# megvii-research/OccDepth

Measured on AMD Instinct MI355X. Metric: frames/sec forward, SemanticKITTI stereo->256x256x32 voxels, higher is better.
Workload: dtype f32 storage and accumulate; matrix arithmetic as 3x bf16 split (hi + mid + lo of both operands, six v_mfma_f32_32x32x16_bf16 per K step; error vs float64 tested within 1.5x of the exact-fp32 kernels', measured 0.8-1.1x) in the head convolutions (K2s3), the small-volume 3x3x3 convolutions and transpo

## Files before the change

include/occdepth_amd.h:

```cpp
#ifndef OCCDEPTH_AMD_H
#define OCCDEPTH_AMD_H

#include <stdint.h>

#ifdef __cplusplus
extern "C" {
#endif

#define OCCD_OK 0
#define OCCD_EINVAL (-1)
#define OCCD_ELAUNCH (-2)
#define OCCD_ENOMEM (-3)

#define OCCD_MAX_VIEWS 4
#define OCCD_MAX_SCALES 4

#define OCCD_ACT_NONE 0
#define OCCD_ACT_RELU 1
#define OCCD_ACT_SIGMOID 2
#define OCCD_ACT_RELU_PRE 3

#define OCCD_ABI_VERSION 22
int occd_abi_version(void);
const char* occd_strerror(int code);
// ... 214 lines not shown
                       float* y, int32_t batch, int32_t C, int32_t H, int32_t W, int32_t k,
                       int32_t stride, int32_t pad_top, int32_t pad_left, int32_t Ho, int32_t Wo,
                       int32_t act, void* stream);
int occd_stem_conv3x3_nchw(const float* x, const float* w, const float* scale, const float* shift, float* y,
                           int32_t batch, int32_t H, int32_t W, int32_t cout, int32_t stride, int32_t pad_top,
                           int32_t pad_left, int32_t Ho, int32_t Wo, int32_t act, void* stream);
int occd_upsample_bilinear_cat_nchw(const float* x, const float* skip, float* out, int32_t batch,
                                    int32_t C, int32_t Cskip, int32_t h, int32_t w, int32_t H,
                                    int32_t W, void* stream);
int occd_upsample_bilinear_cat_nhwc(const float* x, const float* skip, float* out, int32_t batch, int32_t C, int32_t Cskip,
                                    int32_t h, int32_t w, int32_t H, int32_t W, void* stream);
int occd_upsample_bilinear_cat_nhwc_rows(const float* x, const float* skip, float* out, int32_t batch, int32_t C, int32_t Cskip,
                                         int32_t h, int32_t w, int32_t H, int32_t W, int32_t out_cs, void* stream);
int occd_upsample_bilinear_nhwc_bwd(const float* gout, float* gx, int32_t batch, int32_t C, int32_t gout_cs, int32_t h,
                                    int32_t w, int32_t H, int32_t W, void* stream);

int occd_upconv_gather_nchw(const float* z, float* out, int32_t batch, int32_t Cout, int32_t h, int32_t w,
                            int32_t H, int32_t W, int64_t z_channel_stride, int64_t z_batch_stride, void* stream);

int occd_upconv_gather_skip_nchw(const float* z, const float* skip, const float* wskip, const float* shift, float* out,
                                 int32_t batch, int32_t Cout, int32_t Cs, int32_t h, int32_t w, int32_t H, int32_t W,
                                 int64_t z_channel_stride, int64_t z_batch_stride, float slope, void* stream);

int occd_wino_input_transform_nchw(const float* x, float* V, int32_t batch, int32_t Cin, int32_t H, int32_t W,
                                   int32_t ty0, int32_t ths, void* stream);
int occd_wino_output_transform_nchw(const float* M, const float* scale, const float* shift, const float* res,
                                    float* y, int32_t batch, int32_t Cout, int32_t H, int32_t W, int32_t ty0,
                                    int32_t ths, int32_t act, float slope, int32_t res_first, void* stream);

int occd_wino_input_transform_cm(const float* x, float* Vt, int32_t batch, int32_t Cin, int32_t H, int32_t W,
                                 int64_t Tp, void* stream);
int occd_wino_output_transform_cm(const float* Mt, const float* scale, const float* shift, const float* res,
                                  float* y, int32_t batch, int32_t Cout, int32_t H, int32_t W, int64_t Tp,
                                  int32_t act, float slope, int32_t res_first, void* stream);

typedef struct occd_wino_args {
    const float* x;
    const float* upk;
    const float* shift;
    const float* res;
    float* y;
    int32_t batch, cin, cout, H, W;
    int32_t act, res_first, tile_hint;
    float slope;
} occd_wino_args;
int64_t occd_wino_packed_floats(int32_t cout, int32_t cin);
int occd_wino_pack_weights(const float* w, const float* scale, float* upk, int32_t cout, int32_t cin, void* stream);
int occd_wino_conv3x3_fwd(const occd_wino_args* a, void* stream);

int64_t occd_wino_packed_f16x2_bytes(int32_t cout, int32_t cin);
int occd_wino_pack_weights_f16x2(const float* w, const float* scale, void* upk, int32_t cout, int32_t cin, void* stream);
int occd_wino_conv3x3_f16x2_fwd(const occd_wino_args* a, void* stream);
int occd_wino_conv3x3_f16x2_fwd_ex(const occd_wino_args* a, int32_t max_workgroups, void* stream);

int occd_dwconv2d_bwd_data_nchw(const float* gy, const float* w, float* dx, int32_t batch, int32_t C, int32_t H,
                                int32_t W, int32_t k, int32_t stride, int32_t pad_top, int32_t pad_left, int32_t Ho,
                                int32_t Wo, void* stream);
int64_t occd_dwconv2d_bwd_weight_workspace_floats(int32_t batch, int32_t C, int32_t k, int32_t Ho, int32_t Wo);
int occd_dwconv2d_bwd_weight_nchw(const float* x, const float* gy, float* dw, float* workspace, int32_t batch, int32_t C,
                                  int32_t H, int32_t W, int32_t k, int32_t stride, int32_t pad_top, int32_t pad_left,
                                  int32_t Ho, int32_t Wo, void* stream);
int32_t occd_dwconv2d_pool_blocks(int32_t Ho, int32_t Wo);
int occd_dwconv2d_pool_nchw(const float* x, const float* w, const float* scale, const float* shift, float* y,
                            float* pool_part, int32_t batch, int32_t C, int32_t H, int32_t W, int32_t k,
                            int32_t stride, int32_t pad_top, int32_t pad_left, int32_t Ho, int32_t Wo,
                            int32_t act, int64_t x_plane_stride, void* stream);
int32_t occd_dwconv2d_set_stage(int32_t form);
int occd_plane_reduce(const float* a, const float* b, float* out, int64_t planes, int64_t S, void* stream);
int occd_se_bwd(const float* gg, const float* gate, const float* sums, const float* r, const float* w_reduce,
                const float* b_reduce, const float* w_expand, float* dz_scratch, float* gm, float* gw_reduce,
                float* gb_reduce, float* gw_expand, float* gb_expand, int32_t batch, int32_t C, int32_t Cr, int64_t S,
                void* stream);
int occd_depthnet_gate(const float* sps, const float* intrins, int64_t intr_stride, float factor, const float* w1,
                       const float* b1, const float* w2, const float* b2, const float* wr, const float* br,
                       const float* we, const float* be, float* gate, int32_t images, int32_t C, void* stream);
int occd_se_gate(const float* pool_part, const float* w_reduce, const float* b_reduce, const float* w_expand,
                 const float* b_expand, float* r_scratch, float* gate, int32_t batch, int32_t C, int32_t Cr,
                 int32_t nblk, int64_t S, void* stream);
int32_t occd_se_gate_set_fused(int32_t on);

int occd_graph_replace_memsets(void* graph);

typedef struct occd_pw_args {
    const float* x;
    const float* wpk;
    const float* shift;
    const float* gate;
    const float* res;
    float* y;
    int64_t N;
    int32_t batch, cin, cout;
    int32_t act, tile_hint;
    float slope;
    int32_t out_nhwc_cs;
} occd_pw_args;
int64_t occd_pw_packed_floats(int32_t cout, int32_t cin);
int occd_pw_pack_weights(const float* w, const float* scale, float* wpk, int32_t cout, int32_t cin, void* stream);
int occd_pw_conv_fwd(const occd_pw_args* a, void* stream);

int occd_argmax_channels(const float* x, int64_t rows, int32_t cs, int32_t coff, int32_t C,
                         const uint16_t* lut, uint16_t* out, void* stream);

#define OCCD_RENDER_MAX_VIEWS 8
typedef struct OccdRenderView {
    float o0[3], ou[3], ov[3];
    float d0[3], du[3], dv[3];
// ... 617 lines not shown
```

occdepth_amd/csrc/wino_conv2d.hip:

```cpp
#include <atomic>
#include <type_traits>
#include <vector>
#include "device.h"

namespace {

struct WinoP {
    const float* x;
    const float* upk;
    const float* shift;
    const float* res;
    float* y;
    int B, Cin, Cout, H, W;
    int chunks, nblk, wg_ty, wg_tx, nwg;
    int act, res_first;
    float slope;
};

constexpr uint32_t kWinoOutside = 0xFFFFFFF0u;
__device__ __forceinline__ float wino_acc_read(float a) {
    float t;
    asm volatile("v_accvgpr_read_b32 %0, %1" : "=v"(t) : "a"(a));
    return t;
}
// ... 295 lines not shown
    if (i >= total) return;
    const int j = i & 3, lane = (i >> 2) & 63;
    long t = i >> 8;
    const int blk = t % nblk; t /= nblk;
    const int rec = t & 15;
    const int chunk = (int)(t >> 4);
    const int q = rec >> 2, hh = (rec >> 1) & 1, part = rec & 1;
    const int xi = 8 * hh + 4 * part + j;
    const int co = blk * 32 + (lane & 31), ci = chunk * 8 + (lane >> 5) * 4 + q;
    float out = 0.f;
    if (co < cout && ci < cin) {
        const double G[4][3] = {{1, 0, 0}, {0.5, 0.5, 0.5}, {0.5, -0.5, 0.5}, {0, 0, 1}};
        const float* g = w + ((size_t)co * cin + ci) * 9;
        const int a = xi >> 2, bcol = xi & 3;
        double s = 0.0;
#pragma unroll
        for (int m = 0; m < 3; ++m)
#pragma unroll
            for (int n = 0; n < 3; ++n) s += G[a][m] * (double)g[m * 3 + n] * G[bcol][n];
        if (scale != nullptr) s *= (double)scale[co];
        out = (float)s;
    }
    upk[i] = out;
}

constexpr int kWinoStageExp = 1;
typedef _Float16 f16x2 __attribute__((ext_vector_type(2)));

struct WinoHP {
    const float* x;
    const uint16_t* upk;
    const float* fac;
    const float* shift;
    const float* res;
    float* y;
    int B, Cin, Cout, H, W;
    int chunks, nblk, wg_ty, wg_tx, nwg;
    int act, res_first;
    float slope;
};

__device__ __forceinline__ void split2_f16x2(float a, float b, uint32_t& hi, uint32_t& lo) {
    asm("" : "+v"(a));
    asm("" : "+v"(b));
    const f16x2 h = __builtin_convertvector((f32x2){a, b}, f16x2);
    float r0 = __builtin_fmaf((float)h[0], -2048.f, a * 2048.f);
    float r1 = __builtin_fmaf((float)h[1], -2048.f, b * 2048.f);
    asm("" : "+v"(r0));
    asm("" : "+v"(r1));
    hi = __builtin_bit_cast(uint32_t, h);
    lo = __builtin_bit_cast(uint32_t, __builtin_convertvector((f32x2){r0, r1}, f16x2));
}

template <int TWV, bool PERSIST, bool WE>
__global__ void __launch_bounds__(512, 2) wino3x3_f16x2_kernel(const WinoHP p) {
    constexpr int RW = 32 / TWV;
    constexpr int WGR = 4 * RW;
    constexpr int PR = 2 * WGR + 2;
    constexpr int PC = 2 * TWV + 2;
    constexpr int RS = TWV == 16 ? 48 : 68;
    constexpr int PLANE = PR * RS;
    constexpr int NEL = 8 * PLANE;
    constexpr int NDMA = (NEL + 511) / 512;
    constexpr int PBUF = NDMA * 512;
    constexpr int UOFF = 4 * PBUF;
    constexpr int XOFF = PERSIST ? 2 * PBUF : 0;
    constexpr int XFLOATS = 4 * 2 * 64 * 64 / (PERSIST ? 2 : 1);
    static_assert(XOFF + XFLOATS <= (PERSIST ? UOFF + 32 * 256 : 4 * 2 * 64 * 64), "the exchange must fit in the staging buffers");
    static_assert((UOFF + 32 * 256) * 4 <= 160 * 1024 && (XOFF + XFLOATS) * 4 <= 160 * 1024, "LDS of a CU");
    static_assert(XOFF % 4 == 0, "16-byte aligned exchange");
    extern __shared__ __attribute__((aligned(16))) float lds[];

    const size_t plane_hw = (size_t)p.H * p.W;
    const size_t u_rec = (size_t)p.nblk * 512;
    uint32_t voff[NDMA];
    int nb, b, ty0, tx0;
    auto fresh_tid = [] {
        int t = threadIdx.x;
        asm volatile("" : "+v"(t));
        return t;
    };
    const int wave = __builtin_amdgcn_readfirstlane(threadIdx.x >> 6);
    const int pr = wave & 3, h = wave >> 2;
    const bool h0 = h == 0;

    auto setup = [&](uint32_t v) {
        const uint32_t bid = xcd_remap(v, p.nwg);
        nb = bid % p.nblk;
        uint32_t t = bid / p.nblk;
        const int bx = t % p.wg_tx;
        t /= p.wg_tx;
        const int by = t % p.wg_ty;
        b = t / p.wg_ty;
        ty0 = by * WGR, tx0 = bx * TWV;
        const int gy0 = 2 * ty0 - 1, gx0 = 2 * tx0 - 1;
        const int lane = fresh_tid() & 63;
#pragma unroll
        for (int i = 0; i < NDMA; ++i) {
            const int e = (wave * NDMA + i) * 64 + lane;
            const int cin = e / PLANE, rem = e - cin * PLANE;
            const int row = rem / RS, col = rem - row * RS;
            const int gy = gy0 + row, gx = gx0 + col;
            const bool ok = e < NEL && col < PC && (unsigned)gy < (unsigned)p.H && (unsigned)gx < (unsigned)p.W;
            voff[i] = ok ? (uint32_t)((cin * plane_hw + (size_t)gy * p.W + gx) * 4) : 0xFFFFFFF0u;
        }
    };
    auto issue_patch = [&](int c, bool live = true) {
        const float* const xb = p.x + (size_t)b * p.Cin * plane_hw;
#pragma unroll
        for (int s = 0; s < 2; ++s) {
            const int ch0 = c * 16 + s * 8, left = live ? p.Cin - ch0 : 0;
            const auto rsrc = __builtin_amdgcn_make_buffer_rsrc((void*)(xb + (size_t)(left > 0 ? ch0 : 0) * plane_hw), 0,
                                                                left > 0 ? (uint32_t)((size_t)left * plane_hw * 4) : 0u, 0x00020000);
            float* pdst = lds + ((c & 1) * 2 + s) * PBUF + wave * NDMA * 64;
#pragma unroll
            for (int i = 0; i < NDMA; ++i)
                __builtin_amdgcn_raw_ptr_buffer_load_lds(rsrc, pdst + i * 64, 4, voff[i], 0, 0, 0);
        }
    };

    asm volatile("" ::"a"(0.f));
    f32x16 acc[8];

    static_assert(kWinoStageExp == 1, "the transform below stages 2 V");
    auto row_v = [&](auto hc, auto ic, const float* pl, uint32_t (&vh)[4][4], uint32_t (&vl)[4][4]) {
        constexpr int H = decltype(hc)::value, I = decltype(ic)::value;
        constexpr int RA = H == 0 ? I : 1 - I, RB = H == 1 && I == 0 ? 0 : 2;
        constexpr bool ADD = H == 0 && I == 1;
#pragma unroll
        for (int m = 0; m < 4; ++m) {
            float v[2][4];
#pragma unroll
            for (int e = 0; e < 2; ++e) {
                const float* pq = pl + (2 * m + e) * PLANE;
                const f32x2 a0 = *(const f32x2*)(pq + RA * RS), a1 = *(const f32x2*)(pq + RA * RS + 2);
                const f32x2 b0 = *(const f32x2*)(pq + RB * RS), b1 = *(const f32x2*)(pq + RB * RS + 2);
                float ra[4] = {a0.x, a0.y, a1.x, a1.y};
#pragma unroll
                for (int j = 0; j < 4; ++j) asm("" : "+v"(ra[j]));
                const float t0 = ADD ? ra[0] + b0.x : ra[0] - b0.x, t1 = ADD ? ra[1] + b0.y : ra[1] - b0.y;
                const float t2 = ADD ? ra[2] + b1.x : ra[2] - b1.x, t3 = ADD ? ra[3] + b1.y : ra[3] - b1.y;
                const float u1 = 2.f * t1, u2 = 2.f * t2;
                v[e][0] = __builtin_fmaf(2.f, t0, -u2);
                v[e][1] = u1 + u2;
                v[e][2] = u2 - u1;
                v[e][3] = __builtin_fmaf(-2.f, t3, u1);
            }
#pragma unroll
            for (int j = 0; j < 4; ++j) split2_f16x2(v[0][j], v[1][j], vh[j][m], vl[j][m]);
        }
    };
    auto row_m = [&](auto ic, const u32x4* ul, const uint32_t (&vh)[4][4], const uint32_t (&vl)[4][4]) {
        constexpr int I = decltype(ic)::value;
#pragma unroll
        for (int j = 0; j < 4; j += 2) {
            f16x8 uh[2], ulo[2], us[2], bh[2], bl[2];
#pragma unroll
            for (int e = 0; e < 2; ++e) {
                uh[e] = __builtin_bit_cast(f16x8, ul[(2 * (4 * I + j + e)) * 64]);
                ulo[e] = __builtin_bit_cast(f16x8, ul[(2 * (4 * I + j + e) + 1) * 64]);
                us[e] = uh[e] * (_Float16)(1.f / 2048.f);
                bh[e] = __builtin_bit_cast(f16x8, (u32x4){vh[j + e][0], vh[j + e][1], vh[j + e][2], vh[j + e][3]});
                bl[e] = __builtin_bit_cast(f16x8, (u32x4){vl[j + e][0], vl[j + e][1], vl[j + e][2], vl[j + e][3]});
            }
#pragma unroll
            for (int e = 0; e < 2; ++e)
                acc[4 * I + j + e] = __builtin_amdgcn_mfma_f32_32x32x16_f16(ulo[e], bh[e], acc[4 * I + j + e], 0, 0, 0);
#pragma unroll
            for (int e = 0; e < 2; ++e)
                acc[4 * I + j + e] = __builtin_amdgcn_mfma_f32_32x32x16_f16(us[e], bl[e], acc[4 * I + j + e], 0, 0, 0);
#pragma unroll
            for (int e = 0; e < 2; ++e)
                acc[4 * I + j + e] = __builtin_amdgcn_mfma_f32_32x32x16_f16(uh[e], bh[e], acc[4 * I + j + e], 0, 0, 0);
        }
    };
    using I0 = std::integral_constant<int, 0>;
    using I1 = std::integral_constant<int, 1>;

    uint32_t v = blockIdx.x;
    setup(v);
    issue_patch(0);
    for (;;) {
        const int lane = fresh_tid() & 63;
        const int li = lane & 31, kk = lane >> 5;
        const int lr = pr * RW + li / TWV, lc = li % TWV;
        const int pbase = kk * PBUF + (2 * lr + h) * RS + 2 * lc;
        const u32x4* const ul = (const u32x4*)(lds + UOFF) + (h * 16 * 64 + lane);
        const uint16_t* const ubase = p.upk + (size_t)nb * 512 + lane * 8;
        auto issue_u = [&](int c) {
            float* udst = lds + UOFF + wave * 4 * 256;
            const uint16_t* usrc = ubase + ((size_t)c * 32 + wave * 4) * u_rec;
#pragma unroll
            for (int j = 0; j < 4; ++j) __builtin_amdgcn_global_load_lds(usrc + (size_t)j * u_rec, udst + j * 256, 16, 0, 0);
        };
#pragma unroll
        for (int k = 0; k < 8; ++k)
#pragma unroll
            for (int r = 0; r < 16; ++r) acc[k][r] = 0.f;

        __syncthreads();
        for (int c = 0; c < p.chunks; ++c) {
            issue_u(c);
            if (c + 1 < p.chunks) issue_patch(c + 1);
            const float* pl = lds + (c & 1) * 2 * PBUF + pbase;
            uint32_t ah[4][4], al[4][4], bh[4][4], bl[4][4];
            if (h0) row_v(I0{}, I0{}, pl, ah, al);
            else row_v(I1{}, I0{}, pl, ah, al);
            __syncthreads();
            row_m(I0{}, ul, ah, al);
            if (h0) row_v(I0{}, I1{}, pl, bh, bl);
            else row_v(I1{}, I1{}, pl, bh, bl);
            row_m(I1{}, ul, bh, bl);
            __syncthreads();
        }

        const int nb_c = nb, b_c = b, ty0_c = ty0, tx0_c = tx0;
        const uint32_t vn = v + gridDim.x;
        const bool more = PERSIST && vn < (uint32_t)p.nwg;
        wino_exchange_store<TWV, true, PERSIST ? 2 : 1, WE>(p, p.fac, acc, lds + XOFF, h, pr, fresh_tid() & 63, nb_c, b_c, ty0_c, tx0_c, [&] {
            if (PERSIST) {
                setup(more ? vn : v);
                issue_patch(0, more);
            }
        });
        if (!more) {
            if (PERSIST) asm volatile("s_waitcnt vmcnt(0)" ::: "memory");
            break;
        }
        v = vn;
    }
}

__device__ __forceinline__ double wino_u_f64(const float* g, int xi) {
    const double G[4][3] = {{1, 0, 0}, {0.5, 0.5, 0.5}, {0.5, -0.5, 0.5}, {0, 0, 1}};
    const int a = xi >> 2, bcol = xi & 3;
    double s = 0.0;
#pragma unroll
    for (int m = 0; m < 3; ++m)
#pragma unroll
        for (int n = 0; n < 3; ++n) s += G[a][m] * (double)g[m * 3 + n] * G[bcol][n];
    return s;
}

__global__ void wino_f16x2_scale_kernel(const float* __restrict__ w, const float* __restrict__ scale, float* __restrict__ fac,
                                        int cout, int cin, int nblk) {
    const int co = blockIdx.x * blockDim.x + threadIdx.x;
    if (co >= nblk * 32) return;
    double m = 0.0;
    bool bad = false;
    if (co < cout) {
        const double sc = scale != nullptr ? (double)scale[co] : 1.0;
        for (int ci = 0; ci < cin; ++ci)
            for (int xi = 0; xi < 16; ++xi) {
                const double v = fabs(wino_u_f64(w + ((size_t)co * cin + ci) * 9, xi) * sc);
                if (!(v <= 3.0e38)) bad = true;
                m = fmax(m, v);
            }
    }
    int e = 0;
    const bool ok = m > 0.0 && !bad;
    if (ok) frexp(m, &e);
    const int k = ok ? min(max(14 - e, -100), 100) : 0;
    fac[co] = bad ? __builtin_nanf("") : ldexpf(1.f, -(k + kWinoStageExp));
}

__global__ void wino_pack_f16x2_kernel(const float* __restrict__ w, const float* __restrict__ scale,
                                       const float* __restrict__ fac, uint16_t* __restrict__ upk, int cout, int cin, int nblk,
                                       long total) {
    const long i = (long)blockIdx.x * blockDim.x + threadIdx.x;
    if (i >= total) return;
    const int j = i & 7, lane = (i >> 3) & 63;
    long t = i >> 9;
    const int blk = t % nblk; t /= nblk;
    const int img = t & 1, xi = (t >> 1) & 15;
    const int chunk = (int)(t >> 5);
    const int co = blk * 32 + (lane & 31), ci = chunk * 16 + (lane >> 5) * 8 + j;
    float v = 0.f;
    if (co < cout && ci < cin) {
        double s = wino_u_f64(w + ((size_t)co * cin + ci) * 9, xi);
        if (scale != nullptr) s *= (double)scale[co];
        v = (float)(s * (double)(ldexpf(1.f, -kWinoStageExp) / fac[co]));
    }
    const _Float16 hi = (_Float16)v;
    upk[i] = __builtin_bit_cast(uint16_t, img == 0 ? hi : (_Float16)(v - (float)hi));
}

template <int TWV, bool WE, int EXP = 0>
int launch_wino_we(const WinoP& p, hipStream_t st) {
    constexpr int RW = 32 / TWV, PR = 2 * 4 * RW + 2, RS = TWV == 16 ? 48 : 68;
    constexpr int PBUF = (8 * PR * RS + 511) / 512 * 512;
    size_t lds = ((size_t)2 * PBUF + 2 * 16 * 256) * sizeof(float);
    const size_t xchg = (size_t)4 * 2 * 64 * 64 * sizeof(float);
    if (lds < xchg) lds = xchg;
    if (occd::ensure_big_lds(reinterpret_cast<const void*>(wino3x3_kernel<TWV, WE, EXP>)) != OCCD_OK) return OCCD_ELAUNCH;
    hipLaunchKernelGGL((wino3x3_kernel<TWV, WE, EXP>), dim3((unsigned)p.nwg), dim3(512), lds, st, p);
    return occd::check_launch();
}

template <int TWV, bool WE>
int launch_wino_f16x2_we(const WinoHP& p, int grid, hipStream_t st) {
    constexpr int RW = 32 / TWV, PR = 2 * 4 * RW + 2, RS = TWV == 16 ? 48 : 68;
    constexpr int PBUF = (8 * PR * RS + 511) / 512 * 512;
    size_t lds = ((size_t)4 * PBUF + 32 * 256) * sizeof(float);
    if (grid > 0) {
        if (occd::ensure_big_lds(reinterpret_cast<const void*>(wino3x3_f16x2_kernel<TWV, true, WE>)) != OCCD_OK) return OCCD_ELAUNCH;
        hipLaunchKernelGGL((wino3x3_f16x2_kernel<TWV, true, WE>), dim3((unsigned)grid), dim3(512), lds, st, p);
        return occd::check_launch();
    }
    const size_t xchg = (size_t)4 * 2 * 64 * 64 * sizeof(float);
    if (lds < xchg) lds = xchg;
    if (occd::ensure_big_lds(reinterpret_cast<const void*>(wino3x3_f16x2_kernel<TWV, false, WE>)) != OCCD_OK) return OCCD_ELAUNCH;
    hipLaunchKernelGGL((wino3x3_f16x2_kernel<TWV, false, WE>), dim3((unsigned)p.nwg), dim3(512), lds, st, p);
    return occd::check_launch();
}

template <int TWV, int EXP = 0>
int launch_wino(const WinoP& p, hipStream_t st) {
    return (p.W & 1) == 0 ? launch_wino_we<TWV, true, EXP>(p, st) : launch_wino_we<TWV, false, EXP>(p, st);
}

template <int TWV>
int launch_wino_f16x2(const WinoHP& p, int grid, hipStream_t st) {
    return (p.W & 1) == 0 ? launch_wino_f16x2_we<TWV, true>(p, grid, st) : launch_wino_f16x2_we<TWV, false>(p, grid, st);
}

template <class P>
int wino_geometry(const occd_wino_args* a, int cin_step, P& p) {
    if (a == nullptr || a->x == nullptr || a->upk == nullptr || a->y == nullptr) return OCCD_EINVAL;
    if (a->batch < 1 || a->cin < 1 || a->cout < 1 || a->H < 1 || a->W < 1) return OCCD_EINVAL;
    if (a->act < 0 || a->act > 3) return OCCD_EINVAL;
    if ((double)a->cin * a->H * a->W >= 2147483648.0) return OCCD_EINVAL;
    if (20.0 * a->H * a->W >= 4294967040.0) return OCCD_EINVAL;
    p.x = a->x; p.shift = a->shift; p.res = a->res; p.y = a->y;
    p.B = a->batch; p.Cin = a->cin; p.Cout = a->cout; p.H = a->H; p.W = a->W;
    p.chunks = (a->cin + cin_step - 1) / cin_step;
    p.nblk = (a->cout + 31) / 32;
    p.act = a->act; p.res_first = a->res_first; p.slope = a->slope;
    const int th = (a->H + 1) / 2, tw = (a->W + 1) / 2;
    const int hint = a->tile_hint % 100;
    int twv = hint == 16 || hint == 32 ? hint : 0;
    if (twv == 0) {
        const long w16 = (long)((tw + 15) / 16) * 16 * ((th + 7) / 8) * 8;
        const long w32 = (long)((tw + 31) / 32) * 32 * ((th + 3) / 4) * 4;
        twv = w32 <= w16 ? 32 : 16;
    }
    const int wgr = twv == 16 ? 8 : 4;
    p.wg_tx = (tw + twv - 1) / twv;
    p.wg_ty = (th + wgr - 1) / wgr;
    const long nwg = (long)p.nblk * p.wg_tx * p.wg_ty * p.B;
    if (nwg > 0x7fffffffL) return OCCD_EINVAL;
    p.nwg = (int)nwg;
    return twv;
}

int wino_cu_count() {
    static std::atomic<int> cached[64];
    int dev = 0;
    if (hipGetDevice(&dev) != hipSuccess || dev < 0 || dev >= 64) return 0;
    int n = cached[dev].load(std::memory_order_relaxed);
    if (n == 0) {
        if (hipDeviceGetAttribute(&n, hipDeviceAttributeMultiprocessorCount, dev) != hipSuccess || n < 1) return 0;
        cached[dev].store(n, std::memory_order_relaxed);
    }
    return n;
}

// ... 31 lines not shown
    (void)exp_mode;
#endif
    return twv == 16 ? launch_wino<16>(p, (hipStream_t)stream) : launch_wino<32>(p, (hipStream_t)stream);
}

int64_t occd_wino_packed_f16x2_bytes(int32_t cout, int32_t cin) {
    if (cout < 1 || cin < 1) return OCCD_EINVAL;
    const int64_t nblk = (cout + 31) / 32;
    return (int64_t)((cin + 15) / 16) * 32 * nblk * 512 * 2 + nblk * 32 * 4;
}

int occd_wino_pack_weights_f16x2(const float* w, const float* scale, void* upk, int32_t cout, int32_t cin, void* stream) {
    if (w == nullptr || upk == nullptr || cout < 1 || cin < 1) return OCCD_EINVAL;
    const int nblk = (cout + 31) / 32;
    const long total = (long)((cin + 15) / 16) * 32 * nblk * 512;
    float* fac = reinterpret_cast<float*>(static_cast<uint16_t*>(upk) + total);
    hipLaunchKernelGGL(wino_f16x2_scale_kernel, dim3((unsigned)nblk), dim3(32), 0, (hipStream_t)stream, w, scale, fac, cout,
                       cin, nblk);
    hipLaunchKernelGGL(wino_pack_f16x2_kernel, dim3((unsigned)((total + 255) / 256)), dim3(256), 0, (hipStream_t)stream, w,
                       scale, fac, static_cast<uint16_t*>(upk), cout, cin, nblk, total);
    const int rc = occd::check_launch();
    if (rc != OCCD_OK) return rc;
    std::vector<float> host((size_t)nblk * 32);
    if (hipMemcpyAsync(host.data(), fac, host.size() * sizeof(float), hipMemcpyDeviceToHost, (hipStream_t)stream) != hipSuccess ||
        hipStreamSynchronize((hipStream_t)stream) != hipSuccess)
        return OCCD_ELAUNCH;
    for (float f : host)
        if (f != f) return OCCD_EINVAL;
    return OCCD_OK;
}

int occd_wino_conv3x3_f16x2_fwd_ex(const occd_wino_args* a, int32_t max_workgroups, void* stream) {
    if (max_workgroups < -1) return OCCD_EINVAL;
    WinoHP p{};
    const int twv = wino_geometry(a, 16, p);
    if (twv < 0) return twv;
    p.upk = reinterpret_cast<const uint16_t*>(a->upk);
    p.fac = reinterpret_cast<const float*>(p.upk + (size_t)p.chunks * 32 * p.nblk * 512);
    int grid = 0;
    if (max_workgroups > 0) {
        grid = p.nwg < max_workgroups ? p.nwg : max_workgroups;
    } else if (max_workgroups == 0) {
        const int cus = wino_cu_count();
        if (cus < 1) return OCCD_ELAUNCH;
        grid = cus >= 8 ? cus - cus % 8 : cus;
        if (p.nwg <= grid) grid = 0;
    }
    const double tiles = (double)p.B * ((a->H + 1) / 2) * ((a->W + 1) / 2);
    occd::ProfScope prof("wino_conv3x3_f16x2", (hipStream_t)stream, 2.0 * 16 * tiles * ((a->cin + 7) / 8) * 8 * p.nblk * 32,
                         4.0 * p.B * ((double)p.Cin + p.Cout) * p.H * p.W);
    return twv == 16 ? launch_wino_f16x2<16>(p, grid, (hipStream_t)stream) : launch_wino_f16x2<32>(p, grid, (hipStream_t)stream);
}

int occd_wino_conv3x3_f16x2_fwd(const occd_wino_args* a, void* stream) {
    static const int dflt = [] {
        const char* e = getenv("OCCDEPTH_WINO_PERSIST");
        if (e == nullptr || (e[0] == '0' && e[1] == '\0')) return -1;
        return e[0] == '1' && e[1] == '\0' ? 0 : -2;
    }();
    if (dflt < -1) return OCCD_EINVAL;
    return occd_wino_conv3x3_f16x2_fwd_ex(a, dflt, stream);
}

}
```

occdepth_amd/hip.py:

```python
import collections
import ctypes
import os
from ctypes import c_int32, c_int64, c_void_p

import torch

from . import abi

_HERE = os.path.dirname(os.path.abspath(__file__))
LIB_PATH = os.path.join(_HERE, "libocc_hip.so")

EXPORTS = abi.EXPORTS
ABI_VERSION = abi.ABI_VERSION
MAX_VIEWS = abi.CONSTANTS["OCCD_MAX_VIEWS"]
MAX_SCALES = abi.CONSTANTS["OCCD_MAX_SCALES"]
ACT_NONE = abi.CONSTANTS["OCCD_ACT_NONE"]
ACT_RELU = abi.CONSTANTS["OCCD_ACT_RELU"]
ACT_SIGMOID = abi.CONSTANTS["OCCD_ACT_SIGMOID"]
ACT_RELU_PRE = abi.CONSTANTS["OCCD_ACT_RELU_PRE"]
OPTIM_CHUNK = abi.CONSTANTS["OCCD_OPTIM_CHUNK"]
MAX_REGIONS = abi.CONSTANTS["OCCD_MAX_REGIONS"]

Conv3dArgs = abi.STRUCTS["occd_conv3d_args"]
WgradArgs = abi.STRUCTS["occd_conv3d_wgrad_args"]
# ... 1292 lines not shown
    return upk


class WinoF16x2:

    __slots__ = ("image", "cout", "cin", "f32")

    def __init__(self, image, cout, cin, f32=None):
        self.image, self.cout, self.cin, self.f32 = image, cout, cin, f32


_CU_COUNT = {}


def _cu_count(device):
    n = _CU_COUNT.get(device)
    if n is None:
        n = _CU_COUNT[device] = torch.cuda.get_device_properties(device).multi_processor_count
    return n


def wino_f16x2_wins(B, cin, cout, H, W, device=None):
    tiles = B * ((H + 1) // 2) * ((W + 1) // 2)
    return ((cout + 31) // 32) * ((tiles + 127) // 128) >= _cu_count(torch.cuda.current_device() if device is None else device)


def wino_pack_weights_f16x2(w, scale=None):
    cout, cin = w.shape[0], w.shape[1]
    if tuple(w.shape[2:]) != (3, 3):
        raise RuntimeError("wino_pack_weights_f16x2 needs a (Cout, Cin, 3, 3) weight")
    n = load().occd_wino_packed_f16x2_bytes(cout, cin)
    if n <= 0:
        raise RuntimeError("occd_wino_packed_f16x2_bytes: bad shape")
    wc = w.detach().float().contiguous()
    sc = scale.detach().float().contiguous() if scale is not None else None
    image = torch.empty(n, device=w.device, dtype=torch.uint8)
    rc = load().occd_wino_pack_weights_f16x2(_f32(wc, "w"), _f32(sc, "scale") if sc is not None else None,
                                             _ptr(image, "upk"), cout, cin, _stream())
    if rc == -1:
        raise ValueError("wino_pack_weights_f16x2: non-finite weights (keep the float32 image of wino_pack_weights)")
    _check(rc, "occd_wino_pack_weights_f16x2")
    return WinoF16x2(image, cout, cin)


def _parse_wino_persist(value):
    if value not in ("0", "1"):
        raise ValueError("OCCDEPTH_WINO_PERSIST must be 0 or 1, not %r" % (value,))
    return value == "1"


WINO_PERSIST = _parse_wino_persist(os.environ.get("OCCDEPTH_WINO_PERSIST", "0"))


def conv2d_3x3_fused(x, upk, cout, shift=None, act=None, slope=0.01, res=None, res_first=False, tile_hint=0, out=None,
                     max_workgroups=None):
    if not x.is_contiguous():
        x = x.contiguous()
    B, cin, H, W = x.shape
    y = torch.empty((B, cout, H, W), device=x.device, dtype=torch.float32) if out is None else out
    if res is not None and not res.is_contiguous():
        res = res.contiguous()
    if max_workgroups is not None and not isinstance(upk, WinoF16x2):
        raise RuntimeError("max_workgroups is K10h's grid: the operand of this launch is K10's float32 image")
    if isinstance(upk, WinoF16x2) and upk.f32 is not None and not wino_f16x2_wins(B, cin, cout, H, W, x.device):
        upk = upk.f32
    split = isinstance(upk, WinoF16x2)
    a = WinoArgs()
    a.x, a.y = _f32(x, "x"), _f32(y, "y")
    a.upk = _ptr(upk.image, "upk") if split else _f32(upk, "upk")
    a.shift = _f32(shift, "shift") if shift is not None else None
    a.res = _f32(res, "res") if res is not None else None
    a.batch, a.cin, a.cout, a.H, a.W = B, cin, cout, H, W
    a.act, a.res_first, a.tile_hint, a.slope = ACT2D[act], 1 if res_first else 0, int(tile_hint), float(slope)
    if (upk.cout, upk.cin) != (cout, cin) if split else upk.numel() != load().occd_wino_packed_floats(cout, cin):
        raise RuntimeError("packed Winograd weights do not match (cout, cin)")
    if _PROFILING:
        set_tag("%d>%d @%dx%dx%d" % (cin, cout, B, H, W))
    if split:
        if max_workgroups is None:
            max_workgroups = 0 if WINO_PERSIST else -1
        _check(load().occd_wino_conv3x3_f16x2_fwd_ex(ctypes.byref(a), int(max_workgroups), _stream()),
               "occd_wino_conv3x3_f16x2_fwd_ex")
    else:
        _check(load().occd_wino_conv3x3_fwd(ctypes.byref(a), _stream()), "occd_wino_conv3x3_fwd")
    return y


def pw_pack_weights(w, scale=None):
    cout, cin = w.shape[0], w.shape[1]
    n = load().occd_pw_packed_floats(cout, cin)
    if n <= 0 or w.numel() != cout * cin:
        raise RuntimeError("pw_pack_weights needs a (Cout, Cin[, 1, 1]) weight")
    wc = w.detach().float().reshape(cout, cin).contiguous()
    wpk = torch.empty(n, device=w.device, dtype=torch.float32)
    sc = scale.detach().float().contiguous() if scale is not None else None
    _check(load().occd_pw_pack_weights(_f32(wc, "w"), _f32(sc, "scale") if sc is not None else None, _f32(wpk, "wpk"),
                                       cout, cin, _stream()), "occd_pw_pack_weights")
    return wpk


def conv1x1(x, wpk, cout, shift=None, act=None, slope=0.01, gate=None, res=None, tile_hint=0, out=None, nhwc=False):
    if not x.is_contiguous():
        x = x.contiguous()
    B, cin = x.shape[0], x.shape[1]
    sp = tuple(x.shape[2:])
    N = 1
    for d in sp:
        N *= d
    ocs = round_up(cout, 4) if nhwc else 0
    if nhwc:
        y = torch.empty((B,) + sp + (ocs,), device=x.device, dtype=torch.float32)
    else:
        y = torch.empty((B, cout) + sp, device=x.device, dtype=torch.float32) if out is None else out
    if res is not None and not res.is_contiguous():
        res = res.contiguous()
    if gate is not None:
        gate = gate.reshape(B, cin)
        if not gate.is_contiguous():
            gate = gate.contiguous()
    if wpk.numel() != load().occd_pw_packed_floats(cout, cin):
        raise RuntimeError("packed 1x1 weights do not match (cout, cin)")
    a = PwArgs()
    a.x, a.wpk, a.y = _f32(x, "x"), _f32(wpk, "wpk"), _f32(y, "y")
    a.shift = _f32(shift, "shift") if shift is not None else None
    a.gate = _f32(gate, "gate") if gate is not None else None
    a.res = _f32(res, "res") if res is not None else None
    a.N, a.batch, a.cin, a.cout = N, B, cin, cout
    a.act, a.tile_hint, a.slope, a.out_nhwc_cs = ACT2D[act], int(tile_hint), float(slope), ocs
    if _PROFILING:
        set_tag("%d>%d @%dx%d" % (cin, cout, B, N))
    _check(load().occd_pw_conv_fwd(ctypes.byref(a), _stream()), "occd_pw_conv_fwd")
    if nhwc:
        nd = len(sp)
        return y[..., :cout].permute(0, nd + 1, *range(1, nd + 1))
    return y
# ... 2011 lines not shown
```

Measured before the change: 72.38.

## Add cout-pair Winograd f16x2 kernel computing two output-channel blocks per workgroup

Adds a second form of the split-f16 Winograd 3x3 kernel in which each workgroup covers two 32-channel output blocks over half as many tile rows. Each wave transforms one of the four Winograd rows, and the four row results are combined through an LDS exchange before the output transform and store. The input patch transform is therefore shared across two output blocks, cutting redundant input loads and transforms. A shape table picks this form by default for specific batch-2 layer shapes, at the cost of more LDS, an extra exchange step and fewer tile rows per workgroup.

```diff
diff --git a/include/occdepth_amd.h b/include/occdepth_amd.h
--- a/include/occdepth_amd.h
+++ b/include/occdepth_amd.h
@@ -290,6 +290,7 @@
 int occd_wino_pack_weights_f16x2(const float* w, const float* scale, void* upk, int32_t cout, int32_t cin, void* stream);
 int occd_wino_conv3x3_f16x2_fwd(const occd_wino_args* a, void* stream);
 int occd_wino_conv3x3_f16x2_fwd_ex(const occd_wino_args* a, int32_t max_workgroups, void* stream);
+int occd_wino_conv3x3_f16x2_fwd_form(const occd_wino_args* a, int32_t max_workgroups, int32_t cout_blocks, void* stream);
 
 int occd_dwconv2d_bwd_data_nchw(const float* gy, const float* w, float* dx, int32_t batch, int32_t C, int32_t H,
                                 int32_t W, int32_t k, int32_t stride, int32_t pad_top, int32_t pad_left, int32_t Ho,
diff --git a/occdepth_amd/csrc/wino_conv2d.hip b/occdepth_amd/csrc/wino_conv2d.hip
--- a/occdepth_amd/csrc/wino_conv2d.hip
+++ b/occdepth_amd/csrc/wino_conv2d.hip
@@ -371,6 +371,35 @@
     lo = __builtin_bit_cast(uint32_t, __builtin_convertvector((f32x2){r0, r1}, f16x2));
 }
 
+static_assert(kWinoStageExp == 1, "the transform below stages 2 V");
+template <int H, int I, int PLANE, int RS>
+__device__ __forceinline__ void wino_row_v(const float* pl, uint32_t (&vh)[4][4], uint32_t (&vl)[4][4]) {
+    constexpr int RA = H == 0 ? I : 1 - I, RB = H == 1 && I == 0 ? 0 : 2;
+    constexpr bool ADD = H == 0 && I == 1;
+#pragma unroll
+    for (int m = 0; m < 4; ++m) {
+        float v[2][4];
+#pragma unroll
+        for (int e = 0; e < 2; ++e) {
+            const float* pq = pl + (2 * m + e) * PLANE;
+            const f32x2 a0 = *(const f32x2*)(pq + RA * RS), a1 = *(const f32x2*)(pq + RA * RS + 2);
+            const f32x2 b0 = *(const f32x2*)(pq + RB * RS), b1 = *(const f32x2*)(pq + RB * RS + 2);
+            float ra[4] = {a0.x, a0.y, a1.x, a1.y};
+#pragma unroll
+            for (int j = 0; j < 4; ++j) asm("" : "+v"(ra[j]));
+            const float t0 = ADD ? ra[0] + b0.x : ra[0] - b0.x, t1 = ADD ? ra[1] + b0.y : ra[1] - b0.y;
+            const float t2 = ADD ? ra[2] + b1.x : ra[2] - b1.x, t3 = ADD ? ra[3] + b1.y : ra[3] - b1.y;
+            const float u1 = 2.f * t1, u2 = 2.f * t2;
+            v[e][0] = __builtin_fmaf(2.f, t0, -u2);
+            v[e][1] = u1 + u2;
+            v[e][2] = u2 - u1;
+            v[e][3] = __builtin_fmaf(-2.f, t3, u1);
+        }
+#pragma unroll
+        for (int j = 0; j < 4; ++j) split2_f16x2(v[0][j], v[1][j], vh[j][m], vl[j][m]);
+    }
+}
+
 template <int TWV, bool PERSIST, bool WE>
 __global__ void __launch_bounds__(512, 2) wino3x3_f16x2_kernel(const WinoHP p) {
     constexpr int RW = 32 / TWV;
@@ -441,34 +470,6 @@
     asm volatile("" ::"a"(0.f));
     f32x16 acc[8];
 
-    static_assert(kWinoStageExp == 1, "the transform below stages 2 V");
-    auto row_v = [&](auto hc, auto ic, const float* pl, uint32_t (&vh)[4][4], uint32_t (&vl)[4][4]) {
-        constexpr int H = decltype(hc)::value, I = decltype(ic)::value;
-        constexpr int RA = H == 0 ? I : 1 - I, RB = H == 1 && I == 0 ? 0 : 2;
-        constexpr bool ADD = H == 0 && I == 1;
-#pragma unroll
-        for (int m = 0; m < 4; ++m) {
-            float v[2][4];
-#pragma unroll
-            for (int e = 0; e < 2; ++e) {
-                const float* pq = pl + (2 * m + e) * PLANE;
-                const f32x2 a0 = *(const f32x2*)(pq + RA * RS), a1 = *(const f32x2*)(pq + RA * RS + 2);
-                const f32x2 b0 = *(const f32x2*)(pq + RB * RS), b1 = *(const f32x2*)(pq + RB * RS + 2);
-                float ra[4] = {a0.x, a0.y, a1.x, a1.y};
-#pragma unroll
-                for (int j = 0; j < 4; ++j) asm("" : "+v"(ra[j]));
-                const float t0 = ADD ? ra[0] + b0.x : ra[0] - b0.x, t1 = ADD ? ra[1] + b0.y : ra[1] - b0.y;
-                const float t2 = ADD ? ra[2] + b1.x : ra[2] - b1.x, t3 = ADD ? ra[3] + b1.y : ra[3] - b1.y;
-                const float u1 = 2.f * t1, u2 = 2.f * t2;
-                v[e][0] = __builtin_fmaf(2.f, t0, -u2);
-                v[e][1] = u1 + u2;
-                v[e][2] = u2 - u1;
-                v[e][3] = __builtin_fmaf(-2.f, t3, u1);
-            }
-#pragma unroll
-            for (int j = 0; j < 4; ++j) split2_f16x2(v[0][j], v[1][j], vh[j][m], vl[j][m]);
-        }
-    };
     auto row_m = [&](auto ic, const u32x4* ul, const uint32_t (&vh)[4][4], const uint32_t (&vl)[4][4]) {
         constexpr int I = decltype(ic)::value;
 #pragma unroll
@@ -523,12 +524,12 @@
             if (c + 1 < p.chunks) issue_patch(c + 1);
             const float* pl = lds + (c & 1) * 2 * PBUF + pbase;
             uint32_t ah[4][4], al[4][4], bh[4][4], bl[4][4];
-            if (h0) row_v(I0{}, I0{}, pl, ah, al);
-            else row_v(I1{}, I0{}, pl, ah, al);
+            if (h0) wino_row_v<0, 0, PLANE, RS>(pl, ah, al);
+            else wino_row_v<1, 0, PLANE, RS>(pl, ah, al);
             __syncthreads();
             row_m(I0{}, ul, ah, al);
-            if (h0) row_v(I0{}, I1{}, pl, bh, bl);
-            else row_v(I1{}, I1{}, pl, bh, bl);
+            if (h0) wino_row_v<0, 1, PLANE, RS>(pl, bh, bl);
+            else wino_row_v<1, 1, PLANE, RS>(pl, bh, bl);
             row_m(I1{}, ul, bh, bl);
             __syncthreads();
         }
@@ -548,6 +549,269 @@
         }
         v = vn;
     }
+}
+
+template <int TWV, bool WE>
+__device__ __forceinline__ void wino_quad_exchange_store(const WinoHP& p, f32x16 (&acc)[8], float* xchg, int row, int g, int lane,
+                                                         int nb0, bool live1, int b, int ty0, int tx0) {
+    wino_acc_settle(acc);
+    constexpr int RW = 32 / TWV;
+    const int li = lane & 31, kk = lane >> 5;
+    const int lr = g * RW + li / TWV, lc = li % TWV;
+    const int oy0 = 2 * (ty0 + lr), ox = 2 * (tx0 + lc);
+    const size_t hw = (size_t)p.H * p.W;
+    const int cb = nb0 * 32 + 8 * row;
+    auto cout_of = [](int r8) { return 32 * (r8 >> 2) + (r8 & 3); };
+    uint32_t vo[2][2];
+#pragma unroll
+    for (int a = 0; a < 2; ++a) {
+        const bool ok = ox < p.W && oy0 + a < p.H;
+        const uint32_t o = (uint32_t)(((size_t)(4 * kk) * hw + (size_t)(oy0 + a) * p.W + ox) * 4);
+        vo[a][0] = ok ? o : kWinoOutside;
+        vo[a][1] = ok && ox + 1 < p.W ? o + 4 : kWinoOutside;
+    }
+    const size_t plane0 = ((size_t)b * p.Cout + cb) * hw;
+    auto desc = [&](const float* base, int r8) {
+        const int rem = p.Cout - cb - cout_of(r8);
+        const uint32_t n = base == nullptr || rem <= 0 ? 0u : (uint32_t)((size_t)(rem < 5 ? rem : 5) * hw * 4);
+        return __builtin_amdgcn_make_buffer_rsrc((void*)((base == nullptr ? p.y : base) + plane0 + (size_t)cout_of(r8) * hw), 0, n,
+                                                 0x00020000);
+    };
+    float sh[8], fc[8], rn[4];
+    {
+        const auto ss = __builtin_amdgcn_make_buffer_rsrc((void*)(p.shift != nullptr ? p.shift : p.y), 0,
+                                                          p.shift != nullptr ? (uint32_t)p.Cout * 4u : 0u, 0x00020000);
+        const auto fs = __builtin_amdgcn_make_buffer_rsrc((void*)p.fac, 0, (uint32_t)p.Cout * 4u, 0x00020000);
+        const uint32_t co4 = (uint32_t)(cb + 4 * kk) * 4;
+#pragma unroll
+        for (int r8 = 0; r8 < 8; ++r8) {
+            sh[r8] = __builtin_bit_cast(float, __builtin_amdgcn_raw_buffer_load_b32(ss, co4 + cout_of(r8) * 4, 0, 0));
+            fc[r8] = __builtin_bit_cast(float, __builtin_amdgcn_raw_buffer_load_b32(fs, co4 + cout_of(r8) * 4, 0, 0));
+        }
+    }
+    auto res_issue = [&](int r8) {
+        const auto rs = desc(p.res, r8);
+#pragma unroll
+        for (int a = 0; a < 2; ++a) {
+            if (WE) {
+                const u32x2 v = __builtin_amdgcn_raw_buffer_load_b64(rs, vo[a][0], 0, 0);
+                const uint32_t v0 = v[0], v1 = v[1];
+                rn[2 * a] = __builtin_bit_cast(float, v0);
+                rn[2 * a + 1] = __builtin_bit_cast(float, v1);
+            } else {
+                rn[2 * a] = __builtin_bit_cast(float, __builtin_amdgcn_raw_buffer_load_b32(rs, vo[a][0], 0, 0));
+                rn[2 * a + 1] = __builtin_bit_cast(float, __builtin_amdgcn_raw_buffer_load_b32(rs, vo[a][1], 0, 0));
+            }
+        }
+    };
+    res_issue(0);
+    __builtin_amdgcn_sched_barrier(0);
+
+    auto xwrite = [&](auto ic, int blk) {
+        constexpr int I = decltype(ic)::value;
+#pragma unroll
+        for (int j = 0; j < 4; ++j) {
+#pragma unroll
+            for (int rd = 0; rd < 4; ++rd) {
+                if (rd == I) continue;
+                float* dst = xchg + (((g * 4 + rd) * 3 + (I < rd ? I : I - 1)) * 16 + j * 4) * 64 + lane;
+#pragma unroll
+                for (int t = 0; t < 4; ++t) dst[t * 64] = wino_acc_read(acc[blk * 4 + j][4 * rd + t]);
+            }
+            __builtin_amdgcn_sched_barrier(0);
+        }
+    };
+    auto finish = [&](auto ic, int blk) {
+        constexpr int I = decltype(ic)::value;
+        const float* theirs = xchg + ((g * 4 + I) * 3 * 16) * 64 + lane;
+#pragma unroll
+        for (int t = 0; t < 4; ++t) {
+            __builtin_amdgcn_sched_barrier(0);
+            const int r8 = blk * 4 + t;
+            const float rc[4] = {rn[0], rn[1], rn[2], rn[3]};
+            if (r8 + 1 < 8) res_issue(r8 + 1);
+            float m[4][4];
+#pragma unroll
+            for (int i = 0; i < 4; ++i)
+#pragma unroll
+                for (int j = 0; j < 4; ++j)
+                    m[i][j] = i == I ? wino_acc_read(acc[blk * 4 + j][4 * I + t]) : theirs[(((i < I ? i : i - 1) * 16) + j * 4 + t) * 64];
+            float s[2][4];
+#pragma unroll
+            for (int j = 0; j < 4; ++j) {
+                s[0][j] = m[0][j] + m[1][j] + m[2][j];
+                s[1][j] = m[1][j] - m[2][j] - m[3][j];
+            }
+            const auto ws = desc(p.y, r8);
+#pragma unroll
+            for (int a = 0; a < 2; ++a) {
+                float y0 = __builtin_fmaf(s[a][0] + s[a][1] + s[a][2], fc[r8], sh[r8]);
+                float y1 = __builtin_fmaf(s[a][1] - s[a][2] - s[a][3], fc[r8], sh[r8]);
+                const float r0 = rc[2 * a], r1 = rc[2 * a + 1];
+                if (p.res_first) { y0 += r0; y1 += r1; }
+                y0 = act2d_exact(y0, p.act, p.slope);
+                y1 = act2d_exact(y1, p.act, p.slope);
+                if (!p.res_first) { y0 += r0; y1 += r1; }
+                if (WE) {
+                    __builtin_amdgcn_raw_buffer_store_b64((u32x2){__builtin_bit_cast(uint32_t, y0), __builtin_bit_cast(uint32_t, y1)},
+                                                          ws, vo[a][0], 0, 0);
+                } else {
+                    __builtin_amdgcn_raw_buffer_store_b32(__builtin_bit_cast(uint32_t, y0), ws, vo[a][0], 0, 0);
+                    __builtin_amdgcn_raw_buffer_store_b32(__builtin_bit_cast(uint32_t, y1), ws, vo[a][1], 0, 0);
+                }
+            }
+        }
+    };
+    auto by_row = [&](auto f, int blk) {
+        if (row == 0) f(std::integral_constant<int, 0>{}, blk);
+        else if (row == 1) f(std::integral_constant<int, 1>{}, blk);
+        else if (row == 2) f(std::integral_constant<int, 2>{}, blk);
+        else f(std::integral_constant<int, 3>{}, blk);
+    };
+    by_row(xwrite, 0);
+    wino_lds_barrier();
+    by_row(finish, 0);
+    if (live1) {
+        wino_lds_barrier();
+        by_row(xwrite, 1);
+        wino_lds_barrier();
+        by_row(finish, 1);
+    }
+}
+
+template <int TWV, bool WE>
+__global__ void __launch_bounds__(512, 2) wino3x3_f16x2_pair_kernel(const WinoHP p) {
+    constexpr int RW = 32 / TWV;
+    constexpr int WGR = 2 * RW;
+    constexpr int PR = 2 * WGR + 2;
+    constexpr int PC = 2 * TWV + 2;
+    constexpr int RS = TWV == 16 ? 48 : 68;
+    constexpr int PLANE = PR * RS;
+    constexpr int NEL = 8 * PLANE;
+    constexpr int NDMA = (NEL + 511) / 512;
+    constexpr int PBUF = NDMA * 512;
+    constexpr int UOFF = 4 * PBUF;
+    constexpr int XFLOATS = 2 * 4 * 3 * 16 * 64;
+    static_assert((UOFF + 64 * 256) * 4 <= 160 * 1024 && XFLOATS * 4 <= 160 * 1024, "LDS of a CU");
+    extern __shared__ __attribute__((aligned(16))) float lds[];
+
+    const size_t plane_hw = (size_t)p.H * p.W;
+    const size_t u_rec = (size_t)p.nblk * 512;
+    const int npair = (p.nblk + 1) >> 1;
+    uint32_t voff[NDMA];
+    auto fresh_tid = [] {
+        int t = threadIdx.x;
+        asm volatile("" : "+v"(t));
+        return t;
+    };
+    const int wave = __builtin_amdgcn_readfirstlane(threadIdx.x >> 6);
+    const int row = wave & 3, g = wave >> 2;
+
+    const uint32_t bid = xcd_remap(blockIdx.x, p.nwg);
+    const int nb0 = 2 * (int)(bid % npair);
+    const bool live1 = nb0 + 1 < p.nblk;
+    uint32_t t = bid / npair;
+    const int bx = t % p.wg_tx;
+    t /= p.wg_tx;
+    const int by = t % p.wg_ty;
+    const int b = t / p.wg_ty;
+    const int ty0 = by * WGR, tx0 = bx * TWV;
+    {
+        const int gy0 = 2 * ty0 - 1, gx0 = 2 * tx0 - 1;
+        const int lane = fresh_tid() & 63;
+#pragma unroll
+        for (int i = 0; i < NDMA; ++i) {
+            const int e = (wave * NDMA + i) * 64 + lane;
+            const int cin = e / PLANE, rem = e - cin * PLANE;
+            const int prow = rem / RS, col = rem - prow * RS;
+            const int gy = gy0 + prow, gx = gx0 + col;
+            const bool ok = e < NEL && col < PC && (unsigned)gy < (unsigned)p.H && (unsigned)gx < (unsigned)p.W;
+            voff[i] = ok ? (uint32_t)((cin * plane_hw + (size_t)gy * p.W + gx) * 4) : 0xFFFFFFF0u;
+        }
+    }
+    auto issue_patch = [&](int c) {
+        const float* const xb = p.x + (size_t)b * p.Cin * plane_hw;
+#pragma unroll
+        for (int s = 0; s < 2; ++s) {
+            const int ch0 = c * 16 + s * 8, left = p.Cin - ch0;
+            const auto rsrc = __builtin_amdgcn_make_buffer_rsrc((void*)(xb + (size_t)(left > 0 ? ch0 : 0) * plane_hw), 0,
+                                                                left > 0 ? (uint32_t)((size_t)left * plane_hw * 4) : 0u, 0x00020000);
+            float* pdst = lds + ((c & 1) * 2 + s) * PBUF + wave * NDMA * 64;
+#pragma unroll
+            for (int i = 0; i < NDMA; ++i)
+                __builtin_amdgcn_raw_ptr_buffer_load_lds(rsrc, pdst + i * 64, 4, voff[i], 0, 0, 0);
+        }
+    };
+
+    asm volatile("" ::"a"(0.f));
+    f32x16 acc[8];
+
+    auto row_m = [&](auto bc, const u32x4* ul, const uint32_t (&vh)[4][4], const uint32_t (&vl)[4][4]) {
+        constexpr int BLK = decltype(bc)::value;
+#pragma unroll
+        for (int j = 0; j < 4; j += 2) {
+            f16x8 uh[2], ulo[2], us[2], bh[2], bl[2];
+#pragma unroll
+            for (int e = 0; e < 2; ++e) {
+                uh[e] = __builtin_bit_cast(f16x8, ul[(BLK * 32 + 2 * (j + e)) * 64]);
+                ulo[e] = __builtin_bit_cast(f16x8, ul[(BLK * 32 + 2 * (j + e) + 1) * 64]);
+                us[e] = uh[e] * (_Float16)(1.f / 2048.f);
+                bh[e] = __builtin_bit_cast(f16x8, (u32x4){vh[j + e][0], vh[j + e][1], vh[j + e][2], vh[j + e][3]});
+                bl[e] = __builtin_bit_cast(f16x8, (u32x4){vl[j + e][0], vl[j + e][1], vl[j + e][2], vl[j + e][3]});
+            }
+#pragma unroll
+            for (int e = 0; e < 2; ++e)
+                acc[4 * BLK + j + e] = __builtin_amdgcn_mfma_f32_32x32x16_f16(ulo[e], bh[e], acc[4 * BLK + j + e], 0, 0, 0);
+#pragma unroll
+            for (int e = 0; e < 2; ++e)
+                acc[4 * BLK + j + e] = __builtin_amdgcn_mfma_f32_32x32x16_f16(us[e], bl[e], acc[4 * BLK + j + e], 0, 0, 0);
+#pragma unroll
+            for (int e = 0; e < 2; ++e)
+                acc[4 * BLK + j + e] = __builtin_amdgcn_mfma_f32_32x32x16_f16(uh[e], bh[e], acc[4 * BLK + j + e], 0, 0, 0);
+        }
+    };
+
+    issue_patch(0);
+    const int lane = fresh_tid() & 63;
+    const int li = lane & 31, kk = lane >> 5;
+    const int lr = g * RW + li / TWV, lc = li % TWV;
+    const int pbase = kk * PBUF + (2 * lr + (row >> 1)) * RS + 2 * lc;
+    const u32x4* const ul = (const u32x4*)(lds + UOFF) + (row * 8 * 64 + lane);
+    const bool u_live = wave < 4 || live1;
+    const uint16_t* const ubase = p.upk + (size_t)(nb0 + (wave >> 2)) * 512 + lane * 8 + (size_t)((wave & 3) * 8) * u_rec;
+    auto issue_u = [&](int c) {
+        float* udst = lds + UOFF + wave * 8 * 256;
+        const uint16_t* usrc = ubase + (size_t)c * 32 * u_rec;
+        if (u_live) {
+#pragma unroll
+            for (int j = 0; j < 8; ++j) __builtin_amdgcn_global_load_lds(usrc + (size_t)j * u_rec, udst + j * 256, 16, 0, 0);
+        }
+    };
+#pragma unroll
+    for (int k = 0; k < 8; ++k)
+#pragma unroll
+        for (int r = 0; r < 16; ++r) acc[k][r] = 0.f;
+
+    __syncthreads();
+    auto k_loop = [&](auto l1) {
+        for (int c = 0; c < p.chunks; ++c) {
+            issue_u(c);
+            if (c + 1 < p.chunks) issue_patch(c + 1);
+            const float* pl = lds + (c & 1) * 2 * PBUF + pbase;
+            uint32_t vh[4][4], vl[4][4];
+            if (row == 0) wino_row_v<0, 0, PLANE, RS>(pl, vh, vl);
+            else if (row == 1) wino_row_v<0, 1, PLANE, RS>(pl, vh, vl);
+            else if (row == 2) wino_row_v<1, 0, PLANE, RS>(pl, vh, vl);
+            else wino_row_v<1, 1, PLANE, RS>(pl, vh, vl);
+            __syncthreads();
+            row_m(std::integral_constant<int, 0>{}, ul, vh, vl);
+            if (decltype(l1)::value) row_m(std::integral_constant<int, 1>{}, ul, vh, vl);
+            __syncthreads();
+        }
+    };
+    if (live1) k_loop(std::true_type{});
+    else k_loop(std::false_type{});
+    wino_quad_exchange_store<TWV, WE>(p, acc, lds, row, g, fresh_tid() & 63, nb0, live1, b, ty0, tx0);
 }
 
 __device__ __forceinline__ double wino_u_f64(const float* g, int xi) {
@@ -631,6 +895,23 @@
     if (occd::ensure_big_lds(reinterpret_cast<const void*>(wino3x3_f16x2_kernel<TWV, false, WE>)) != OCCD_OK) return OCCD_ELAUNCH;
     hipLaunchKernelGGL((wino3x3_f16x2_kernel<TWV, false, WE>), dim3((unsigned)p.nwg), dim3(512), lds, st, p);
     return occd::check_launch();
+}
+
+template <int TWV, bool WE>
+int launch_wino_f16x2_pair_we(const WinoHP& p, hipStream_t st) {
+    constexpr int RW = 32 / TWV, PR = 2 * 2 * RW + 2, RS = TWV == 16 ? 48 : 68;
+    constexpr int PBUF = (8 * PR * RS + 511) / 512 * 512;
+    size_t lds = ((size_t)4 * PBUF + 64 * 256) * sizeof(float);
+    const size_t xchg = (size_t)2 * 4 * 3 * 16 * 64 * sizeof(float);
+    if (lds < xchg) lds = xchg;
+    if (occd::ensure_big_lds(reinterpret_cast<const void*>(wino3x3_f16x2_pair_kernel<TWV, WE>)) != OCCD_OK) return OCCD_ELAUNCH;
+    hipLaunchKernelGGL((wino3x3_f16x2_pair_kernel<TWV, WE>), dim3((unsigned)p.nwg), dim3(512), lds, st, p);
+    return occd::check_launch();
+}
+
+template <int TWV>
+int launch_wino_f16x2_pair(const WinoHP& p, hipStream_t st) {
+    return (p.W & 1) == 0 ? launch_wino_f16x2_pair_we<TWV, true>(p, st) : launch_wino_f16x2_pair_we<TWV, false>(p, st);
 }
 
 template <int TWV, int EXP = 0>
@@ -768,6 +1049,26 @@
     return twv == 16 ? launch_wino_f16x2<16>(p, grid, (hipStream_t)stream) : launch_wino_f16x2<32>(p, grid, (hipStream_t)stream);
 }
 
+int occd_wino_conv3x3_f16x2_fwd_form(const occd_wino_args* a, int32_t max_workgroups, int32_t cout_blocks, void* stream) {
+    if (cout_blocks != 1 && cout_blocks != 2) return OCCD_EINVAL;
+    if (cout_blocks == 1) return occd_wino_conv3x3_f16x2_fwd_ex(a, max_workgroups, stream);
+    if (max_workgroups != -1) return OCCD_EINVAL;
+    WinoHP p{};
+    const int twv = wino_geometry(a, 16, p);
+    if (twv < 0) return twv;
+    p.upk = reinterpret_cast<const uint16_t*>(a->upk);
+    p.fac = reinterpret_cast<const float*>(p.upk + (size_t)p.chunks * 32 * p.nblk * 512);
+    const int th = (a->H + 1) / 2, wgr = twv == 16 ? 4 : 2;
+    p.wg_ty = (th + wgr - 1) / wgr;
+    const long nwg = (long)((p.nblk + 1) / 2) * p.wg_tx * p.wg_ty * p.B;
+    if (nwg > 0x7fffffffL) return OCCD_EINVAL;
+    p.nwg = (int)nwg;
+    const double tiles = (double)p.B * th * ((a->W + 1) / 2);
+    occd::ProfScope prof("wino_conv3x3_f16x2", (hipStream_t)stream, 2.0 * 16 * tiles * ((a->cin + 7) / 8) * 8 * p.nblk * 32,
+                         4.0 * p.B * ((double)p.Cin + p.Cout) * p.H * p.W);
+    return twv == 16 ? launch_wino_f16x2_pair<16>(p, (hipStream_t)stream) : launch_wino_f16x2_pair<32>(p, (hipStream_t)stream);
+}
+
 int occd_wino_conv3x3_f16x2_fwd(const occd_wino_args* a, void* stream) {
     static const int dflt = [] {
         const char* e = getenv("OCCDEPTH_WINO_PERSIST");
diff --git a/occdepth_amd/hip.py b/occdepth_amd/hip.py
--- a/occdepth_amd/hip.py
+++ b/occdepth_amd/hip.py
@@ -1368,8 +1368,24 @@
 WINO_PERSIST = _parse_wino_persist(os.environ.get("OCCDEPTH_WINO_PERSIST", "0"))
 
 
+def _parse_wino_cout_pair(value):
+    if value not in ("auto", "0", "1"):
+        raise ValueError("OCCDEPTH_WINO_COUT_PAIR must be auto, 0 or 1, not %r" % (value,))
+    return None if value == "auto" else value == "1"
+
+
+WINO_COUT_PAIR = _parse_wino_cout_pair(os.environ.get("OCCDEPTH_WINO_COUT_PAIR", "auto"))
+
+WINO_COUT_PAIR_TABLE = frozenset({(160, 160, 185, 610), (320, 320, 93, 305), (128, 128, 47, 153), (32, 160, 185, 610),
+                                  (48, 320, 93, 305), (224, 1280, 24, 77), (80, 640, 47, 153), (64, 128, 47, 153)})
+
+
+def wino_cout_pair_wins(B, cin, cout, H, W):
+    return B == 2 and (cin, cout, H, W) in WINO_COUT_PAIR_TABLE
+
+
 def conv2d_3x3_fused(x, upk, cout, shift=None, act=None, slope=0.01, res=None, res_first=False, tile_hint=0, out=None,
-                     max_workgroups=None):
+                     max_workgroups=None, cout_blocks=None):
     if not x.is_contiguous():
         x = x.contiguous()
     B, cin, H, W = x.shape
@@ -1378,6 +1394,8 @@
         res = res.contiguous()
     if max_workgroups is not None and not isinstance(upk, WinoF16x2):
         raise RuntimeError("max_workgroups is K10h's grid: the operand of this launch is K10's float32 image")
+    if cout_blocks is not None and not isinstance(upk, WinoF16x2):
+        raise RuntimeError("cout_blocks is K10h's work item: the operand of this launch is K10's float32 image")
     if isinstance(upk, WinoF16x2) and upk.f32 is not None and not wino_f16x2_wins(B, cin, cout, H, W, x.device):
         upk = upk.f32
     split = isinstance(upk, WinoF16x2)
@@ -1394,9 +1412,12 @@
         set_tag("%d>%d @%dx%dx%d" % (cin, cout, B, H, W))
     if split:
         if max_workgroups is None:
-            max_workgroups = 0 if WINO_PERSIST else -1
-        _check(load().occd_wino_conv3x3_f16x2_fwd_ex(ctypes.byref(a), int(max_workgroups), _stream()),
-               "occd_wino_conv3x3_f16x2_fwd_ex")
+            max_workgroups = 0 if WINO_PERSIST and cout_blocks != 2 else -1
+        if cout_blocks is None:
+            pair = wino_cout_pair_wins(B, cin, cout, H, W) if WINO_COUT_PAIR is None else WINO_COUT_PAIR
+            cout_blocks = 2 if pair and max_workgroups == -1 else 1
+        _check(load().occd_wino_conv3x3_f16x2_fwd_form(ctypes.byref(a), int(max_workgroups), int(cout_blocks), _stream()),
+               "occd_wino_conv3x3_f16x2_fwd_form")
     else:
         _check(load().occd_wino_conv3x3_fwd(ctypes.byref(a), _stream()), "occd_wino_conv3x3_fwd")
     return y
```

Measured after the change: 73.24 (median of 6 runs). +1.2%, better.
